# sebasv/lp

Measured on NVIDIA B200. Metric: ipm_iterations_per_s, higher is better.
Workload: dtype f64

## Files before the change

lp_b200/csrc/cholesky.cu:

```cuda
#include <nccl.h>

#include <algorithm>
#include <cstring>
#include <mutex>
#include <type_traits>

#include "dist_schedule.hpp"
#include "kernels.hpp"
#include "panel_factor.cuh"

namespace lpb {

namespace {

constexpr int NB = 128;
constexpr int LDS = NB + 1;
constexpr int TRSM_ROWS = 64;

__global__ void __launch_bounds__(512)
potf2_kernel(double* __restrict__ Mat, int64_t ldm, int k0, int nb, int* __restrict__ info) {
  extern __shared__ double S[];
  double* diag = S + NB * LDS;
  const int tx = threadIdx.x, ty = threadIdx.y, tid = ty * 32 + tx;
  double* blk = Mat + (int64_t)k0 * ldm + k0;
  for (int i = ty; i < nb; i += 16)
    for (int k = tx; k <= i; k += 32) S[i * LDS + k] = blk[(int64_t)i * ldm + k];
  __syncthreads();

  for (int j = 0; j < nb; ++j) {
    const double ajj = S[j * LDS + j];
    if (!(ajj > 0.0) || !isfinite(ajj)) {
      if (tid == 0 && *info == 0) *info = k0 + j + 1;
      for (int i = j + tid; i < nb; i += 512) diag[i] = __longlong_as_double(0x7ff8000000000000ll);
      break;
    }
    const double d = sqrt(ajj);
    if (tid == 0) diag[j] = d;
    if (tid < nb - j - 1) S[(j + 1 + tid) * LDS + j] /= d;
    __syncthreads();
    for (int i = j + 1 + ty; i < nb; i += 16) {
      const double lij = S[i * LDS + j];
      for (int k = j + 1 + tx; k <= i; k += 32) S[i * LDS + k] -= lij * S[k * LDS + j];
    }
    __syncthreads();
  }
  __syncthreads();
  for (int i = ty; i < nb; i += 16)
    for (int k = tx; k <= i; k += 32) blk[(int64_t)i * ldm + k] = (k == i) ? diag[i] : S[i * LDS + k];
}

constexpr int SB = 16;
constexpr int NSB = NB / SB;
constexpr int XDP = SB + 1;
constexpr int TWP = 9;

__device__ __forceinline__ void complete_block_inverse(double* S, const double* rdiag, double* Tw, int tid) {
  const int lane = tid & 31, warp = tid >> 5;
  const int b = warp >> 1, h = warp & 1;
  const int ii = lane & 15, cg = lane >> 4;
  double* tw = Tw + warp * SB * TWP;
  for (int d = 1; d < NSB; ++d) {
    if (b < NSB - d) {
      const int j = b, i = b + d;
      const int ccb = 8 * h + 4 * cg;
      double acc[4] = {0.0, 0.0, 0.0, 0.0};
      const double* lrow = S + (i * SB + ii) * LDS;
#pragma unroll
      for (int l = 0; l < SB; ++l) {
        const double lv = lrow[j * SB + l];
#pragma unroll
        for (int e = 0; e < 4; ++e) {
          const int cc = ccb + e;
          const double up = S[(j * SB + cc) * LDS + j * SB + l];
          const double xv = (l > cc) ? up : ((l == cc) ? rdiag[j * SB + cc] : 0.0);
          acc[e] += lv * xv;
        }
      }
      for (int k = j + 1; k < i; ++k) {
#pragma unroll
        for (int l = 0; l < SB; ++l) {
          const double lv = lrow[k * SB + l];
#pragma unroll
          for (int e = 0; e < 4; ++e) acc[e] += lv * S[(j * SB + ccb + e) * LDS + k * SB + l];
        }
      }
#pragma unroll
      for (int e = 0; e < 4; ++e) tw[ii * TWP + 4 * cg + e] = acc[e];
      __syncwarp();
      double o[4] = {0.0, 0.0, 0.0, 0.0};
#pragma unroll
// ... 1307 lines not shown
  return once.run([](int) -> int {
  LPB_TRY(set_smem(potf2_kernel, kPotf2Smem));
  LPB_TRY(set_smem(potf2_inv_kernel, kPotf2InvSmem));
  LPB_TRY(set_smem(trsm_kernel, kTrsmSmem));
  LPB_TRY(set_smem(trsm_blocked_kernel, kTrsmBlockedSmem));
  LPB_TRY(set_smem(trsm_dmma_blocked_kernel, kTrsmDmmaSmem));
  LPB_TRY(set_smem(trsv_diag_kernel<false, 1>, kTrsvSmem));
  LPB_TRY(set_smem(trsv_diag_kernel<false, 2>, kTrsvSmem));
  LPB_TRY(set_smem(trsv_diag_kernel<true, 1>, kTrsvSmem));
  LPB_TRY(set_smem(trsv_diag_kernel<true, 2>, kTrsvSmem));
  return LPB_OK;
  });
}

#define LPB_KCHECK(lc)             \
  do {                             \
    (lc).launches++;               \
    LPB_CUDA(cudaGetLastError());  \
  } while (0)

}

struct CholWs {
  int64_t nblk, ldy, off_y, off_flags, off_wt, off_xt, total;
  explicit CholWs(int64_t m) {
    nblk = ceil_div(m, NB);
    ldy = round_up(m, 2);
    off_y = nblk * NB * NB;
    off_flags = off_y + 2 * ldy;
    off_wt = off_flags + round_up(nblk, 2);
    off_xt = off_wt + nblk * 2 * NB * 2;
    total = off_xt + nblk * 2 * NB * 2;
  }
};

static int ensure_chol_ws(LaunchCtx& lc, int64_t m) {
  const int64_t need = CholWs(m).total;
  if (lc.chol_ws_cap >= need) return LPB_OK;
  if (lc.chol_ws) cudaFree(lc.chol_ws);
  lc.chol_ws = nullptr;
  lc.chol_ws_cap = 0;
  lc.linv_valid_m = -1;
  void* p = nullptr;
  LPB_CUDA(cudaMalloc(&p, sizeof(double) * (size_t)need));
  LPB_CUDA(cudaMemsetAsync(p, 0, sizeof(double) * (size_t)need, lc.stream));
  lc.chol_ws = static_cast<double*>(p);
  lc.chol_ws_cap = need;
  return LPB_OK;
}

static int finish_factor(LaunchCtx& lc, int64_t m, double* Mat, int64_t ldm) {
  if (lc.potf2_impl == 1) {
    lc.linv_valid_m = -1;
    lc.linv_mat = nullptr;
    return LPB_OK;
  }
  if (!lc.linv_full) {
    static PerDeviceOnce once;
    LPB_TRY(once.run([](int) -> int { return set_smem(linv_complete_kernel, kLinvCompleteSmem); }));
    linv_complete_kernel<<<(unsigned)ceil_div(m, NB), dim3(32, 16), kLinvCompleteSmem, lc.stream>>>(Mat, ldm, m, lc.chol_ws);
    LPB_KCHECK(lc);
    lc.linv_full = true;
  }
  lc.linv_valid_m = m;
  lc.linv_mat = Mat;
  return LPB_OK;
}

static int k_potrf_dist(LaunchCtx& lc, int64_t m, double* Mat, int64_t ldm);
static int k_potrf_dist2(LaunchCtx& lc, int64_t m, double* Mat, int64_t ldm);

static int k_potrf_lookahead(LaunchCtx& lc, int64_t m, double* Mat, int64_t ldm) {
  if (!lc.side_stream) {
    int lo = 0, hi = 0;
    LPB_CUDA(cudaDeviceGetStreamPriorityRange(&lo, &hi));
    LPB_CUDA(cudaStreamCreateWithPriority(&lc.side_stream, cudaStreamNonBlocking, hi));
    for (int e = 0; e < 2; ++e) {
      LPB_CUDA(cudaEventCreateWithFlags(&lc.ev_col[e], cudaEventDisableTiming));
      LPB_CUDA(cudaEventCreateWithFlags(&lc.ev_pan[e], cudaEventDisableTiming));
    }
  }
  const int T = (int)ceil_div(m, NB);
  lc.linv_full = false;
  auto nb_of = [&](int k) { return (int)((m - (int64_t)k * NB) < NB ? (m - (int64_t)k * NB) : NB); };
  auto potf2 = [&](int k, cudaStream_t st) -> int {
    potf2_inv_kernel<<<1, dim3(32, 16), kPotf2InvSmem, st>>>(Mat, ldm, k * NB, nb_of(k), lc.info_dev,
                                                             lc.chol_ws + (int64_t)k * NB * NB, 0);
    LPB_KCHECK(lc);
    return LPB_OK;
  };
  auto trsm = [&](int k) -> int {
    const int64_t rem = m - (int64_t)k * NB - nb_of(k);
    if (rem <= 0) return LPB_OK;
    trsm_dmma_blocked_kernel<<<(unsigned)ceil_div(rem, TBR), 256, kTrsmDmmaSmem, lc.stream>>>(
        Mat, ldm, k * NB, (int)m, lc.chol_ws + (int64_t)k * NB * NB);
    LPB_KCHECK(lc);
    return LPB_OK;
  };
  LPB_TRY(potf2(0, lc.stream));
  LPB_TRY(trsm(0));
  const int saved_cap = lc.update_grid_cap;
  int rc = LPB_OK;
  for (int k = 0; k + 1 < T && rc == LPB_OK; ++k) {
    const int64_t k0 = (int64_t)k * NB;
    cudaEvent_t ec = lc.ev_col[k & 1], ep = lc.ev_pan[k & 1];
    rc = k_trailing_update_part(lc, m, Mat, ldm, k0, NB, k + 1, 1, 1, 0);
    if (rc != LPB_OK) break;
    LPB_CUDA(cudaEventRecord(ec, lc.stream));
    LPB_CUDA(cudaStreamWaitEvent(lc.side_stream, ec, 0));
    rc = potf2(k + 1, lc.side_stream);
    if (rc != LPB_OK) break;
    LPB_CUDA(cudaEventRecord(ep, lc.side_stream));
    lc.update_grid_cap = kNumSMs - 1;
    rc = k_trailing_update_part(lc, m, Mat, ldm, k0, NB, k + 2, 0, 1, 0);
    lc.update_grid_cap = saved_cap;
    if (rc != LPB_OK) break;
    LPB_CUDA(cudaStreamWaitEvent(lc.stream, ep, 0));
    rc = trsm(k + 1);
  }
  lc.update_grid_cap = saved_cap;
  LPB_TRY(rc);
  return finish_factor(lc, m, Mat, ldm);
}

int k_potrf(LaunchCtx& lc, int64_t m, double* Mat, int64_t ldm, int syrk_impl) {
  LPB_TRY(configure_once());
  LPB_TRY(ensure_chol_ws(lc, m));
  if (lc.ws_m != m) {
    const CholWs ws(m);
    LPB_CUDA(cudaMemsetAsync(lc.chol_ws + ws.off_flags, 0, sizeof(double) * (size_t)(ws.total - ws.off_flags), lc.stream));
    lc.ws_m = m;
  }
  LPB_CUDA(cudaMemsetAsync(lc.info_dev, 0, sizeof(int), lc.stream));
  const bool dmma_update = lc.update_impl == 0 || lc.update_impl == 2 || lc.update_impl == 6;
  if (lc.world > 1 && lc.nccl_comm && lc.potrf_dist && syrk_impl == 0 && lc.trsm_impl == 0 && dmma_update &&
      lc.potf2_impl == 0 && m > NB && !(ldm & 1) && !(reinterpret_cast<uintptr_t>(Mat) & 15))
    return lc.potrf_dist == 2 ? k_potrf_dist2(lc, m, Mat, ldm) : k_potrf_dist(lc, m, Mat, ldm);
  if (lc.potrf_lookahead && syrk_impl == 0 && lc.trsm_impl == 0 && dmma_update && lc.potf2_impl == 0 &&
      !lc.sync_each_launch && m > 2 * NB && !(ldm & 1) && !(reinterpret_cast<uintptr_t>(Mat) & 15))
    return k_potrf_lookahead(lc, m, Mat, ldm);
  const int full_inverse = lc.trsm_impl == 2 ? 1 : 0;
  lc.linv_full = full_inverse != 0;
  for (int64_t k0 = 0; k0 < m; k0 += NB) {
    const int nb = (int)((m - k0) < NB ? (m - k0) : NB);
    const int64_t rem = m - k0 - nb;
    double* linv = lc.chol_ws + (k0 / NB) * NB * NB;
    if (lc.potf2_impl == 1)
      potf2_kernel<<<1, dim3(32, 16), kPotf2Smem, lc.stream>>>(Mat, ldm, (int)k0, nb, lc.info_dev);
    else
      potf2_inv_kernel<<<1, dim3(32, 16), kPotf2InvSmem, lc.stream>>>(Mat, ldm, (int)k0, nb, lc.info_dev, linv,
                                                                      full_inverse);
    LPB_KCHECK(lc);
    if (lc.sync_each_launch) LPB_CUDA(cudaStreamSynchronize(lc.stream));
    if (rem > 0) {
      if (syrk_impl == 1 || lc.trsm_impl == 1) {
        trsm_kernel<<<(unsigned)ceil_div(rem, TRSM_ROWS), dim3(32, 8), kTrsmSmem, lc.stream>>>(Mat, ldm, (int)k0, nb,
                                                                                               (int)m);
        LPB_KCHECK(lc);
      } else if (lc.trsm_impl == 2) {
        LPB_TRY(k_trsm_dmma(lc, m, Mat, ldm, k0, linv));
      } else if (lc.trsm_impl == 3 || (ldm & 1) || (reinterpret_cast<uintptr_t>(Mat) & 15)) {
        trsm_blocked_kernel<<<(unsigned)ceil_div(rem, TBR), 256, kTrsmBlockedSmem, lc.stream>>>(Mat, ldm, (int)k0,
                                                                                               (int)m, linv);
        LPB_KCHECK(lc);
      } else {
        trsm_dmma_blocked_kernel<<<(unsigned)ceil_div(rem, TBR), 256, kTrsmDmmaSmem, lc.stream>>>(Mat, ldm, (int)k0,
                                                                                                 (int)m, linv);
        LPB_KCHECK(lc);
      }
      if (lc.sync_each_launch) LPB_CUDA(cudaStreamSynchronize(lc.stream));
      if (syrk_impl == 1 || lc.update_impl == 1)
        LPB_TRY(k_trailing_update_simple(lc, m, Mat, ldm, k0, nb));
      else
        LPB_TRY(k_trailing_update_dmma(lc, m, Mat, ldm, k0, nb));
      if (lc.sync_each_launch) LPB_CUDA(cudaStreamSynchronize(lc.stream));
    }
  }
  return finish_factor(lc, m, Mat, ldm);
}

static int ensure_dist_streams(LaunchCtx& lc) {
  if (!lc.side_stream) {
    int lo = 0, hi = 0;
    LPB_CUDA(cudaDeviceGetStreamPriorityRange(&lo, &hi));
    LPB_CUDA(cudaStreamCreateWithPriority(&lc.side_stream, cudaStreamNonBlocking, hi));
    for (int e = 0; e < 2; ++e) {
      LPB_CUDA(cudaEventCreateWithFlags(&lc.ev_col[e], cudaEventDisableTiming));
      LPB_CUDA(cudaEventCreateWithFlags(&lc.ev_pan[e], cudaEventDisableTiming));
    }
  }
  for (int e = 0; e < 4; ++e)
    if (!lc.ev_dist[e]) LPB_CUDA(cudaEventCreateWithFlags(&lc.ev_dist[e], cudaEventDisableTiming));
  return LPB_OK;
}

constexpr int kPushCtasPerPeer = 4;
constexpr int kRingHeaderDoubles = 128;
struct PeerPush {
  double* dst[LaunchCtx::kMaxPeers - 1];
  unsigned long long* flag[LaunchCtx::kMaxPeers - 1];
  int n;
};
__global__ void __launch_bounds__(256)
peer_push_kernel(const double* __restrict__ src, int64_t count2, PeerPush pp, unsigned long long value,
// ... 507 lines not shown
```

lp_b200/csrc/common.cuh:

```cuda
#pragma once
#include <cuda_runtime.h>
#include <cstdint>
#include <cstdio>
#include <cstring>
#include <mutex>

#include "../../include/lpb200.h"

namespace lpb {

void set_last_error(const char* fmt, ...);
const char* get_last_error();

#define LPB_CUDA(call)                                                                         \
  do {                                                                                         \
    cudaError_t e__ = (call);                                                                  \
    if (e__ != cudaSuccess) {                                                                  \
      ::lpb::set_last_error("%s:%d %s -> %s", __FILE__, __LINE__, #call, cudaGetErrorString(e__)); \
      return LPB_ERR_CUDA;                                                                     \
    }                                                                                          \
  } while (0)

#define LPB_TRY(call)              \
  do {                             \
    int rc__ = (call);             \
    if (rc__ != LPB_OK) return rc__; \
  } while (0)

constexpr int kNumSMs = 148;

constexpr int kMaxDevices = 64;
struct PerDeviceOnce {
  std::mutex mu;
  bool done[kMaxDevices] = {};
  template <class F>
  int run(F&& f) {
    int dev = 0;
    LPB_CUDA(cudaGetDevice(&dev));
    if (dev < 0 || dev >= kMaxDevices) return f(dev);
    std::lock_guard<std::mutex> g(mu);
    if (done[dev]) return LPB_OK;
    const int rc = f(dev);
    if (rc == LPB_OK) done[dev] = true;
    return rc;
  }
};

inline int64_t round_up(int64_t v, int64_t a) { return (v + a - 1) / a * a; }
inline int64_t ceil_div(int64_t a, int64_t b) { return (a + b - 1) / b; }

constexpr int kMaxRedVals = 8;
constexpr int kMaxRedBlocks = 1024;
enum RedOp : int { kRedSum = 0, kRedMin = 1 };

struct LaunchCtx {
  cudaStream_t stream = nullptr;
  int64_t launches = 0;
  double* red_partials = nullptr;
  double* red_out = nullptr;
  double* red_host = nullptr;
  unsigned long long* fault_dev = nullptr;
  double* gemv_partials = nullptr;
  int64_t gemv_partials_cap = 0;
  double* chol_ws = nullptr;
  int64_t chol_ws_cap = 0;
  int64_t ws_m = -1;
  int64_t linv_valid_m = -1;
  const double* linv_mat = nullptr;
  bool linv_full = false;
  int solve_epoch = 0;
  int solve_impl = 0;
  int sync_each_launch = 0;
  int syrk_flush_blocks = 32;
  int syrk_tail_split = 1;
  double* syrk_ws = nullptr;
  int64_t syrk_ws_cap = 0;
  int syrk_chain = 0;
  int potf2_impl = 0;
  int trsm_impl = 0, update_impl = 0;
  int solve_grid_cap = 0;
  void* nccl_comm = nullptr;
  int rank = 0, world = 1;
  int potrf_dist = 2;
  double* panel_buf = nullptr;
  int64_t panel_buf_cap = 0;
  int potrf_lookahead = 1;
  cudaStream_t side_stream = nullptr;
  cudaEvent_t ev_col[2] = {nullptr, nullptr}, ev_pan[2] = {nullptr, nullptr};
  bool launch_on_side = false;
  cudaEvent_t ev_dist[4] = {nullptr, nullptr, nullptr, nullptr};
  double* panel_slot[2] = {nullptr, nullptr};
  int64_t panel_slot_cap = 0;
  static constexpr int kMaxPeers = 8;
  double* ring_base = nullptr;
  int64_t ring_slot_doubles = 0;
  int ring_slots = 0;
  double* peer_base[kMaxPeers] = {};
  bool peer_mapped = false;
  bool peer_ready = false;
  uint32_t dist_epoch = 0;
  int update_grid_cap = 0;
  int* info_dev = nullptr;
  int* info_host = nullptr;
};

}
```

lp_b200/csrc/dist_schedule.hpp:

```cpp
#pragma once
#include <cmath>

#if defined(__CUDACC__)
#define LPB_SCHED_HD __host__ __device__
#else
#define LPB_SCHED_HD
#endif

namespace lpb {

struct OwnedCols {
  int G, f, n;
  LPB_SCHED_HD int before(int l) const { return l * (n - f) - G * (l * (l - 1) / 2); }
  LPB_SCHED_HD int count() const {
    if (f >= n) return 0;
    const int nown = (n - f + G - 1) / G;
    return before(nown);
  }
  LPB_SCHED_HD void decode(int t, int* ti, int* tj) const {
    const double a = 0.5 * G, b = (n - f) + 0.5 * G;
    const double disc = b * b - 4.0 * a * t;
    int l = static_cast<int>((b - sqrt(disc > 0.0 ? disc : 0.0)) / (2.0 * a));
    if (l < 0) l = 0;
    while (l > 0 && before(l) > t) --l;
    while (before(l + 1) <= t) ++l;
    *tj = f + l * G;
    *ti = *tj + (t - before(l));
  }
  static LPB_SCHED_HD OwnedCols make(int G, int rank, int tile0, int ntr) {
    OwnedCols o;
    o.G = G;
    o.f = ((rank - tile0) % G + G) % G;
    o.n = ntr;
    return o;
  }
};

template <class Ops>
int potrf_dist_schedule(int T, int G, int me, Ops& ops) {
  int pending = -1;
  for (int k = 0; k < T; ++k) {
    const int owner = k % G;
    int rc;
    if (owner == me && (rc = ops.factor_panel(k)) != 0) return rc;
    if ((rc = ops.broadcast(k, owner)) != 0) return rc;
    if (owner != me && (rc = ops.store_panel(k)) != 0) return rc;
    if (pending >= 0) {
      if ((rc = ops.update_owned(pending, pending + 2)) != 0) return rc;
      pending = -1;
    }
    if (k + 1 < T) {
      if ((k + 1) % G == me) {
        if ((rc = ops.update_column(k, k + 1)) != 0) return rc;
        pending = k;
      } else if ((rc = ops.update_owned(k, k + 1)) != 0) {
        return rc;
      }
    }
  }
  return 0;
}

enum { kEvSmall = 0, kEvPotf2 = 2, kNumDistEvents = 4 };

template <class Ops>
int potrf_dist_schedule2(int T, int G, int me, Ops& ops) {
#define LPB_S2(call)            \
  do {                          \
    const int rc__ = (call);    \
    if (rc__ != 0) return rc__; \
  } while (0)
  int pending = -1;
  for (int k = 0; k < T; ++k) {
    const int owner = k % G;
    if (owner == me) {
      if (k == 0)
        LPB_S2(ops.potf2(0, 0));
      else
        LPB_S2(ops.wait(kEvPotf2 + (k & 1), 0));
      LPB_S2(ops.trsm(k));
    }
    if (k + 1 < T) {
      LPB_S2(ops.bcast_small(k, owner));
      LPB_S2(ops.record(kEvSmall + (k & 1), 0));
    }
    LPB_S2(ops.bcast_large(k, owner));
    if (pending >= 0) {
      LPB_S2(ops.update_owned(pending, pending + 2));
      if (pending % G != me) LPB_S2(ops.unpack(pending));
      pending = -1;
    }
    if (k + 1 < T && (k + 1) % G == me) {
      LPB_S2(ops.wait(kEvSmall + (k & 1), 1));
      LPB_S2(ops.update_diag(k, k + 1, 1));
      LPB_S2(ops.potf2(k + 1, 1));
      LPB_S2(ops.record(kEvPotf2 + ((k + 1) & 1), 1));
      LPB_S2(ops.update_col_below(k, k + 1));
      pending = k;
    } else {
      if (k + 1 < T) LPB_S2(ops.update_owned(k, k + 1));
// ... 10 lines not shown
```

lp_b200/csrc/dmma_gemm.cu:

```cuda
#include <cuda.h>

#include "dist_schedule.hpp"
#include "kernels.hpp"

namespace lpb {

namespace {

constexpr int BM = 128, BN = 128, BK = 16;
constexpr int kStages = 5;
constexpr int kLead = 3;
constexpr int kFlushBlocks = 128;
constexpr int kConsumerWarps = 8;
constexpr int kThreads = kConsumerWarps * 32;
constexpr uint32_t kTileBytes = BM * BK * 8;
constexpr uint32_t kDBytes = BK * 8;
constexpr uint32_t kSmemA = 0;
constexpr uint32_t kSmemB = kSmemA + kStages * kTileBytes;
constexpr uint32_t kSmemD = kSmemB + kStages * kTileBytes;
constexpr uint32_t kSmemBar = kSmemD + kStages * kDBytes;
constexpr uint32_t kSmemTotal = kSmemBar + 2 * kStages * 8;
constexpr uint32_t kSmemAlloc = kSmemTotal + 1024;

template <int MODE, int VAR>
// ... 37 lines not shown
      "{\n\t.reg .pred p;\n\t"
      "mbarrier.try_wait.parity.shared::cta.b64 p, [%1], %2;\n\t"
      "selp.u32 %0, 1, 0, p;\n\t}"
      : "=r"(ok)
      : "r"(bar), "r"(parity)
      : "memory");
  return ok;
}
__device__ __forceinline__ void mbar_wait(uint32_t bar, uint32_t parity) {
  if (mbar_try_wait(bar, parity)) return;
  const long long t0 = clock64();
  while (!mbar_try_wait(bar, parity)) {
    if (clock64() - t0 > 8000000000ll) __trap();
  }
}
__device__ __forceinline__ void tma_load_2d(uint32_t dst, const CUtensorMap* tm, int c0, int c1, uint32_t bar) {
  asm volatile(
      "cp.async.bulk.tensor.2d.shared::cluster.global.mbarrier::complete_tx::bytes [%0], [%1, {%2, %3}], [%4];" ::"r"(
          dst),
      "l"(reinterpret_cast<uint64_t>(tm)), "r"(c0), "r"(c1), "r"(bar)
      : "memory");
}
__device__ __forceinline__ double2 lds_v2(uint32_t addr) {
  double2 v;
  asm volatile("ld.volatile.shared.v2.f64 {%0, %1}, [%2];" : "=d"(v.x), "=d"(v.y) : "r"(addr));
  return v;
}
__device__ __forceinline__ void cp_async_16(uint32_t dst, const void* src) {
  asm volatile("cp.async.cg.shared.global [%0], [%1], 16;" ::"r"(dst), "l"(src) : "memory");
}
__device__ __forceinline__ void cp_async_commit() { asm volatile("cp.async.commit_group;" ::: "memory"); }
__device__ __forceinline__ void cp_async_wait_all() { asm volatile("cp.async.wait_group 0;" ::: "memory"); }
__device__ __forceinline__ void dmma884(double& c0, double& c1, double a, double b) {
  asm("mma.sync.aligned.m8n8k4.row.col.f64.f64.f64.f64 {%0, %1}, {%2}, {%3}, {%0, %1};"
      : "+d"(c0), "+d"(c1)
      : "d"(a), "d"(b));
}

__device__ __forceinline__ void tri_decode(int L, int* ti, int* tj) {
  int i = static_cast<int>((sqrt(8.0 * static_cast<double>(L) + 1.0) - 1.0) * 0.5);
  while (i * (i + 1) / 2 > L) --i;
  while ((i + 1) * (i + 2) / 2 <= L) ++i;
  *ti = i;
  *tj = L - i * (i + 1) / 2;
}

constexpr int kBand = 12;
__device__ __forceinline__ void band_decode(int L, int ntr, int* ti, int* tj) {
  int row, col;
  tri_decode(L, &row, &col);
  const int r0 = (row / kBand) * kBand;
  const int r1 = r0 + kBand < ntr ? r0 + kBand : ntr;
  const int h = r1 - r0;
  int off = L - r0 * (r0 + 1) / 2;
  const int rect = (r0 + 1) * h;
  if (off < rect) {
    *tj = off / h;
    *ti = r0 + off % h;
    return;
  }
  off -= rect;
  int c = r0 + 1, hh = h - 1;
  while (off >= hh) {
    off -= hh;
    ++c;
    --hh;
  }
  *tj = c;
  *ti = c + off;
}

struct LoadCursor {
  int L, kb, row_i, row_j, stage;
  int kb_lo, kb_n;
  uint32_t phase;
};

struct TailSplit {
  int n_full, nsplit;
  double* ws;
};

enum { MODE_SYRK = 0, MODE_UPDATE = 1, MODE_TRSM = 2 };
enum { SHAPE_TRI = 0, SHAPE_COL = 1, SHAPE_OWNED = 2, SHAPE_COLB = 3 };

template <int MODE, bool SCALE, int VAR = 0>
__global__ void __maxnreg__(255)
syrk_dmma_kernel(const __grid_constant__ CUtensorMap tmA, const __grid_constant__ CUtensorMap tmB,
                 double* __restrict__ C, int64_t ldc, int m_total, int tile0, int ntr, int k_begin, int nkb,
                 int col_origin, int shape, OwnedCols own, int p_row0, TailSplit ts) {
  using P = Plan<MODE, VAR>;
  constexpr bool FLUSH = (VAR & 16) == 0;
  constexpr int NS = P::kNS, LEAD = P::kLd;
  constexpr bool CPF = P::kCpf;
  extern __shared__ uint8_t smem_raw[];
  const uint32_t smem_base = (smem_u32(smem_raw) + 1023u) & ~1023u;
  const uint32_t sA = smem_base + P::kA, sB = smem_base + P::kB, sD = smem_base + P::kD, sC = smem_base + P::kC;
  const uint32_t bar_full = smem_base + P::kBar, bar_empty = bar_full + NS * 8;
  const uint32_t bar_cfull = bar_empty + NS * 8, bar_cempty = bar_cfull + 8;
  const uint32_t sF = smem_base + P::kF + threadIdx.x * 16u;

  const int warp = threadIdx.x >> 5, lane = threadIdx.x & 31;
  if (threadIdx.x == 0) {
    for (int s = 0; s < NS; ++s) {
      mbar_init(bar_full + s * 8, 1);
      mbar_init(bar_empty + s * 8, kConsumerWarps);
    }
    mbar_init(bar_cfull, 1);
    mbar_init(bar_cempty, kConsumerWarps);
    asm volatile("fence.mbarrier_init.release.cluster;" ::: "memory");
  }
  __syncthreads();

  constexpr bool SPLIT = MODE == MODE_SYRK && FLUSH && (VAR & 32) != 0;
  const int ntiles_whole = (MODE == MODE_TRSM || shape == SHAPE_COL) ? ntr
                     : (shape == SHAPE_COLB ? ntr - 1 : (shape == SHAPE_OWNED ? own.count() : ntr * (ntr + 1) / 2));
  const int ntiles = SPLIT ? ts.n_full + (ntiles_whole - ts.n_full) * ts.nsplit : ntiles_whole;
  auto item = [&](int I, int* L, int* part, int* kb_lo, int* kb_n) {
    if (!SPLIT || I < ts.n_full) {
      *L = I;
      *part = -1;
      *kb_lo = 0;
      *kb_n = nkb;
    } else {
      const int q = I - ts.n_full;
      *L = ts.n_full + q / ts.nsplit;
      *part = q % ts.nsplit;
      *kb_lo = (int)((int64_t)nkb * *part / ts.nsplit);
      *kb_n = (int)((int64_t)nkb * (*part + 1) / ts.nsplit) - *kb_lo;
    }
  };
  const bool is_producer = threadIdx.x == 0;
  constexpr uint32_t kBytes = 2 * kTileBytes + (SCALE ? kDBytes : 0);

  auto decode = [&](int L, int* ti, int* tj) {
    if (MODE == MODE_TRSM || shape == SHAPE_COL) {
      *ti = L;
      *tj = 0;
    } else if (shape == SHAPE_COLB) {
      *ti = L + 1;
      *tj = 0;
    } else if (shape == SHAPE_OWNED) {
      own.decode(L, ti, tj);
    } else if (MODE == MODE_SYRK) {
      band_decode(L, ntr, ti, tj);
    } else {
      tri_decode(L, ti, tj);
    }
  };

  LoadCursor pc;
  pc.L = blockIdx.x;
  pc.kb = 0;
  pc.stage = 0;
  pc.phase = 0;
  pc.row_i = pc.row_j = 0;
  pc.kb_lo = 0;
  pc.kb_n = nkb;
  auto cursor_tile = [&]() {
    if (pc.L < ntiles) {
      int ti, tj, Lt, part;
      item(pc.L, &Lt, &part, &pc.kb_lo, &pc.kb_n);
      decode(Lt, &ti, &tj);
      pc.row_i = (tile0 + ti) * BM;
      pc.row_j = MODE == MODE_TRSM ? 0 : (tile0 + tj) * BN;
    }
  };
  auto produce_one = [&]() {
    if (pc.L >= ntiles) return;
    mbar_wait(bar_empty + pc.stage * 8, pc.phase ^ 1u);
    const uint32_t full = bar_full + pc.stage * 8;
    mbar_expect_tx(full, kBytes);
    const int k = k_begin + (pc.kb_lo + pc.kb) * BK;
    int ra = pc.row_i, rb = pc.row_j;
    if (MODE == MODE_UPDATE && p_row0 >= 0) {
      ra -= p_row0;
      rb -= p_row0;
      if (ra == BM) ra = 0;
      if (rb == BN) rb = 0;
    }
    tma_load_2d(sA + pc.stage * kTileBytes, &tmA, k, ra, full);
    if (MODE == MODE_TRSM)
      tma_load_2d(sB + pc.stage * kTileBytes, &tmB, (pc.kb_lo + pc.kb) * BK, 0, full);
    else
      tma_load_2d(sB + pc.stage * kTileBytes, &tmA, k, rb, full);
    if (SCALE) tma_load_2d(sD + pc.stage * kDBytes, &tmB, k, 0, full);
    if (++pc.stage == NS) {
      pc.stage = 0;
      pc.phase ^= 1u;
    }
    if (++pc.kb == pc.kb_n) {
      pc.kb = 0;
      pc.L += gridDim.x;
      cursor_tile();
    }
  };
  int c_next = blockIdx.x;
  int c_issued = 0;
  auto produce_c = [&]() {
    if (!CPF || c_next >= ntiles) return;
    if (c_issued > 0) mbar_wait(bar_cempty, static_cast<uint32_t>((c_issued - 1) & 1));
    int ti, tj;
    decode(c_next, &ti, &tj);
    const int r0 = (tile0 + ti) * BM, c0 = (tile0 + tj) * BN;
    mbar_expect_tx(bar_cfull, 8 * kTileBytes);
#pragma unroll
    for (int b = 0; b < 8; ++b) tma_load_2d(sC + b * kTileBytes, &tmB, c0 + b * BK, r0, bar_cfull);
    c_next += gridDim.x;
    ++c_issued;
  };
  if (is_producer) {
    cursor_tile();
    produce_c();
    for (int i = 0; i < LEAD; ++i) produce_one();
  }

  int stage = 0;
  uint32_t phase = 0;
  const int wm = warp >> 2, wn = warp & 3;
  const int g = lane >> 2, t = lane & 3;
  const uint32_t offA = static_cast<uint32_t>(wm * 64 + g) * 128u;
  const uint32_t offB = static_cast<uint32_t>(wn * 32 + g) * 128u;
  const uint32_t sw[2] = {static_cast<uint32_t>(((2 * t + 0) ^ g) << 4), static_cast<uint32_t>(((2 * t + 1) ^ g) << 4)};
  const uint32_t dof[2] = {static_cast<uint32_t>((2 * t + 0) << 4), static_cast<uint32_t>((2 * t + 1) << 4)};

  const int fblocks = MODE == MODE_SYRK && col_origin >= 32 ? col_origin : kFlushBlocks;
  const int fstride = fblocks >> 3;
// ... 279 lines not shown
  if (d)
    LPB_TRY(make_tmap(&tmD, d, 1, (uint64_t)n, (uint64_t)round_up(n, 2), 1, BK, false));
  else
    tmD = tmA;
  const int ntr = (int)ceil_div(m, BM);
  const int nkb = (int)ceil_div(n, BK);
  if (lc.syrk_chain) {
    if (d) return launch_dmma<MODE_SYRK, true, 16>(lc, tmA, tmD, Cmat, ldc, (int)m, 0, ntr, 0, nkb, 0);
    return launch_dmma<MODE_SYRK, false, 16>(lc, tmA, tmD, Cmat, ldc, (int)m, 0, ntr, 0, nkb, 0);
  }
  const int fb = lc.syrk_flush_blocks;
  TailSplit ts{0, 1, nullptr};
  const int ntiles = ntr * (ntr + 1) / 2;
  const int rem = ntiles % kNumSMs;
  if (lc.syrk_tail_split && ntiles > kNumSMs && rem > 0 && 4 * rem <= 3 * kNumSMs && nkb >= 64 && !(m & 1)) {
    int best_s = 1;
    double best = 1.0;
    for (int sp = 2; sp <= 8; ++sp) {
      const double len = (double)ceil_div((int64_t)rem * sp, (int64_t)kNumSMs) / sp + 0.01 * sp;
      if (len < best - 1e-9) {
        best = len;
        best_s = sp;
      }
    }
    if (best_s > 1) {
      const int64_t need = (int64_t)rem * best_s * BM * BN;
      if (lc.syrk_ws_cap < need) {
        if (lc.syrk_ws) LPB_CUDA(cudaFree(lc.syrk_ws));
        lc.syrk_ws = nullptr;
        lc.syrk_ws_cap = 0;
        void* p = nullptr;
        LPB_CUDA(cudaMalloc(&p, sizeof(double) * (size_t)need));
        lc.syrk_ws = static_cast<double*>(p);
        lc.syrk_ws_cap = need;
      }
      ts = TailSplit{ntiles - rem, best_s, lc.syrk_ws};
    }
  }
  if (ts.nsplit > 1) {
    if (d)
      LPB_TRY((launch_dmma<MODE_SYRK, true, 32>(lc, tmA, tmD, Cmat, ldc, (int)m, 0, ntr, 0, nkb, fb, SHAPE_TRI, OwnedCols{1, 0, 0}, -1, ts)));
    else
      LPB_TRY((launch_dmma<MODE_SYRK, false, 32>(lc, tmA, tmD, Cmat, ldc, (int)m, 0, ntr, 0, nkb, fb, SHAPE_TRI, OwnedCols{1, 0, 0}, -1, ts)));
  } else if (d) {
    LPB_TRY((launch_dmma<MODE_SYRK, true>(lc, tmA, tmD, Cmat, ldc, (int)m, 0, ntr, 0, nkb, fb)));
  } else {
    LPB_TRY((launch_dmma<MODE_SYRK, false>(lc, tmA, tmD, Cmat, ldc, (int)m, 0, ntr, 0, nkb, fb)));
  }
  if (ts.nsplit > 1) {
    syrk_tail_fixup_kernel<<<rem, 256, 0, lc.stream>>>(Cmat, ldc, (int)m, ntr, ts);
    lc.launches++;
    LPB_CUDA(cudaGetLastError());
  }
  return LPB_OK;
}

int k_trailing_update_dmma(LaunchCtx& lc, int64_t m, double* Mat, int64_t ldm, int64_t k0, int64_t kb) {
  const int64_t row0 = k0 + kb;
  if (row0 >= m) return LPB_OK;
  if ((row0 % BM) || (kb % BK) || (ldm & 1) || (reinterpret_cast<uintptr_t>(Mat) & 15)) {
    set_last_error("trailing_update_dmma: panel origin must be a multiple of %d, width a multiple of %d", BM, BK);
    return LPB_ERR_BAD_ARGUMENT;
  }
  CUtensorMap tm;
  LPB_TRY(make_tmap(&tm, Mat, (uint64_t)m, (uint64_t)m, (uint64_t)ldm, BM, BK, true));
  const int ntr = (int)ceil_div(m - row0, BM);
  if (lc.update_impl == 2)
    return launch_dmma<MODE_UPDATE, false, 1>(lc, tm, tm, Mat, ldm, (int)m, (int)(row0 / BM), ntr, (int)k0,
                                              (int)(kb / BK), 0);
  if (lc.update_impl == 3)
    return launch_dmma<MODE_UPDATE, false, 2>(lc, tm, tm, Mat, ldm, (int)m, (int)(row0 / BM), ntr, (int)k0,
                                              (int)(kb / BK), 0);
  if (lc.update_impl == 4)
    return launch_dmma<MODE_UPDATE, false, 4>(lc, tm, tm, Mat, ldm, (int)m, (int)(row0 / BM), ntr, (int)k0,
                                              (int)(kb / BK), 0);
  if (lc.update_impl == 5)
    return launch_dmma<MODE_UPDATE, false, 6>(lc, tm, tm, Mat, ldm, (int)m, (int)(row0 / BM), ntr, (int)k0,
                                              (int)(kb / BK), 0);
  return launch_dmma<MODE_UPDATE, false>(lc, tm, tm, Mat, ldm, (int)m, (int)(row0 / BM), ntr, (int)k0, (int)(kb / BK),
                                         0);
}

int k_trailing_update_part(LaunchCtx& lc, int64_t m, double* Mat, int64_t ldm, int64_t k0, int64_t kb, int tile0,
                           int single_col, int own_mod, int own_rem, const double* packed, int64_t packed_rows) {
  int ntr = (int)ceil_div(m, BM) - tile0;
  if (ntr <= 0) return LPB_OK;
  if ((kb % BK) || (ldm & 1) || (reinterpret_cast<uintptr_t>(Mat) & 15) || (int64_t)tile0 * BM < k0 + kb) {
    set_last_error("trailing_update_part: bad panel / tile origin");
    return LPB_ERR_BAD_ARGUMENT;
  }
  CUtensorMap tm, tmc;
  int k_begin = (int)k0, p_row0 = -1;
  LPB_TRY(make_tmap(&tmc, Mat, (uint64_t)m, (uint64_t)m, (uint64_t)ldm, BM, BK, true));
  if (packed) {
    LPB_TRY(make_tmap(&tm, packed, (uint64_t)packed_rows, (uint64_t)BN, (uint64_t)BN, BM, BK, true));
    k_begin = 0;
    p_row0 = (int)k0;
  } else {
    tm = tmc;
  }
  int shape = SHAPE_TRI;
  if (single_col == 1) shape = SHAPE_COL;
  if (single_col == 2) {
    shape = SHAPE_COL;
    ntr = 1;
  }
  if (single_col == 3) shape = SHAPE_COLB;
  if (!single_col && own_mod > 1) shape = SHAPE_OWNED;
  const OwnedCols own = shape == SHAPE_OWNED ? OwnedCols::make(own_mod, own_rem, tile0, ntr) : OwnedCols{1, 0, 0};
  if (lc.update_impl == 2)
    return launch_dmma<MODE_UPDATE, false, 1>(lc, tm, tm, Mat, ldm, (int)m, tile0, ntr, k_begin, (int)(kb / BK), 0, shape,
                                              own, p_row0);
  if (lc.update_impl == 6)
    return launch_dmma<MODE_UPDATE, false, 8>(lc, tm, tmc, Mat, ldm, (int)m, tile0, ntr, k_begin, (int)(kb / BK), 0,
                                              shape, own, p_row0);
  return launch_dmma<MODE_UPDATE, false>(lc, tm, tm, Mat, ldm, (int)m, tile0, ntr, k_begin, (int)(kb / BK), 0, shape, own,
                                         p_row0);
}

int k_trsm_dmma(LaunchCtx& lc, int64_t m, double* Mat, int64_t ldm, int64_t k0, const double* Linv) {
  const int64_t row0 = k0 + BN;
  if (row0 >= m) return LPB_OK;
  if ((row0 % BM) || (ldm & 1) || (reinterpret_cast<uintptr_t>(Mat) & 15) || (reinterpret_cast<uintptr_t>(Linv) & 15)) {
    set_last_error("trsm_dmma: panel origin must be a multiple of %d", BM);
    return LPB_ERR_BAD_ARGUMENT;
  }
  CUtensorMap tm, tl;
  LPB_TRY(make_tmap(&tm, Mat, (uint64_t)m, (uint64_t)m, (uint64_t)ldm, BM, BK, true));
  LPB_TRY(make_tmap(&tl, Linv, (uint64_t)BN, (uint64_t)BN, (uint64_t)BN, BN, BK, true));
  const int ntr = (int)ceil_div(m - row0, BM);
  return launch_dmma<MODE_TRSM, false>(lc, tm, tl, Mat, ldm, (int)m, (int)(row0 / BM), ntr, (int)k0, BN / BK, (int)k0);
}

__global__ void __launch_bounds__(256)
dmma_peak_kernel(double* out, int iters, double a0, double b0) {
  double c[32][2];
#pragma unroll
  for (int i = 0; i < 32; ++i) c[i][0] = c[i][1] = threadIdx.x * 1e-3 + i;
  const double a = a0 + threadIdx.x * 1e-9, b = b0;
  for (int it = 0; it < iters; ++it) {
#pragma unroll
    for (int i = 0; i < 32; ++i) dmma884(c[i][0], c[i][1], a, b);
  }
  double s = 0.0;
#pragma unroll
  for (int i = 0; i < 32; ++i) s += c[i][0] + c[i][1];
  if (s == 12345.678) out[0] = s;
}

int k_dmma_peak(LaunchCtx& lc, double seconds, double* tflops) {
  if (seconds < 0.05) seconds = 0.05;
  if (seconds > 2.0) seconds = 2.0;
  const int iters = 4000;
  const double flop_per_launch = 2.0 * 256 * 32 * iters * 8.0 * kNumSMs;
  cudaEvent_t e0, e1;
  LPB_CUDA(cudaEventCreate(&e0));
  LPB_CUDA(cudaEventCreate(&e1));
  auto run = [&](int launches, float* ms) -> int {
    LPB_CUDA(cudaEventRecord(e0, lc.stream));
    for (int i = 0; i < launches; ++i) dmma_peak_kernel<<<kNumSMs, 256, 0, lc.stream>>>(lc.red_partials, iters, 1.0000001, 1e-9);
    LPB_CUDA(cudaEventRecord(e1, lc.stream));
    LPB_CUDA(cudaEventSynchronize(e1));
    LPB_CUDA(cudaEventElapsedTime(ms, e0, e1));
    lc.launches += launches;
    return LPB_OK;
  };
  float ms = 0.f;
  int rc = run(4, &ms);
  if (rc == LPB_OK) {
    int launches = (int)(seconds * 1e3 / (ms / 4.0 > 1e-3 ? ms / 4.0 : 1e-3));
    if (launches < 8) launches = 8;
    if (launches > 4000) launches = 4000;
    rc = run(launches, &ms);
    if (rc == LPB_OK && tflops) *tflops = flop_per_launch * launches / (ms * 1e-3) * 1e-12;
  }
  cudaEventDestroy(e0);
  cudaEventDestroy(e1);
  return rc;
}

template <bool ACCUM>
__global__ void __launch_bounds__(256)
syrk_simple_kernel(int m_total, int row_origin, int k_begin, int k_end, const double* __restrict__ A, int64_t lda,
                   const double* __restrict__ d, double* __restrict__ C, int64_t ldc) {
  __shared__ double sa[16][65], sb[16][65];
  const int bi = blockIdx.y, bj = blockIdx.x;
  if (bj > bi) return;
  const int tx = threadIdx.x & 15, ty = threadIdx.x >> 4, tid = threadIdx.x;
  double acc[4][4];
#pragma unroll
  for (int i = 0; i < 4; ++i)
#pragma unroll
// ... 62 lines not shown
```

lp_b200/csrc/kernels.hpp:

```cpp
#pragma once
#include "common.cuh"

namespace lpb {

struct RedSpec {
  int nvals = 0;
  int nblocks[kMaxRedVals] = {0};
  int op[kMaxRedVals] = {0};
};
int reduce_finalize(LaunchCtx& lc, const RedSpec& spec);
int fetch_scalars(LaunchCtx& lc, int nvals);

int k_fill(LaunchCtx& lc, double* p, int64_t n, double v);
int k_copy(LaunchCtx& lc, double* dst, const double* src, int64_t n);
int k_dinv(LaunchCtx& lc, int64_t n, const double* x, const double* z, double* dinv);

int k_rhat(LaunchCtx& lc, int64_t n, int mode, double eta, double gm, double a2, double s, const double* x,
           const double* z, const double* rD, const double* dx, const double* dz, double* xs, double* r1);

int k_assemble_delta_n(LaunchCtx& lc, int64_t n, double d_tau, const double* u, const double* p, const double* xs,
                       const double* x, const double* z, double* dx, double* dz, int val_base, int* nblocks);
int k_assemble_delta_m(LaunchCtx& lc, int64_t m, double d_tau, const double* v, const double* q, double* dy);
int k_step(LaunchCtx& lc, int64_t n, double alpha, int clamp, double* x, const double* dx);
int k_extract_x(LaunchCtx& lc, int64_t n, double tau, const double* x, const double* c, double* xo, int val,
                int* nblocks);

int k_resid_p(LaunchCtx& lc, int64_t m, double tau, const double* b, const double* t, const double* y, double* rP,
              int val_base, int* nblocks);
int k_sym_fwd_rhs(LaunchCtx& lc, int64_t m, double eta, const double* rP, const double* b, const double* t0,
                  const double* t1, double* rhs0, double* rhs1, int with_pq);
int k_refine_rhs(LaunchCtx& lc, int64_t m, double eta, const double* rP, const double* b, const double* au,
                 const double* ap, double* rho0, double* rho1, int with_pq);
int k_add_inplace(LaunchCtx& lc, int64_t count, const double* x, double* y);
int k_dots_m(LaunchCtx& lc, int64_t m, const double* b, const double* v, const double* q, int with_pq, int val_base,
             int* nblocks);

int k_gemv_n(LaunchCtx& lc, int64_t m, int64_t n, const double* A, int64_t lda, const double* dinv, const double* w0,
             const double* w1, double* t0, double* t1, int nrhs);
int k_gemv_t_partials(LaunchCtx& lc, int64_t m, int64_t n, const double* A, int64_t lda, const double* v0,
                      const double* v1, int nrhs, int* nchunks);
struct TailCols {
  int64_t nd;
  const int* col_row;
  const double* col_val;
  const double* v0;
  const double* v1;
};
int k_gemv_t_raw(LaunchCtx& lc, int64_t n, int nchunks, int nrhs, double* out0, double* out1);
int k_resid_d(LaunchCtx& lc, int64_t n, int nchunks, double tau, const double* c, const double* z, const double* x,
              double* rD, int val_base, int* nblocks, const TailCols* tail = nullptr);
int k_sym_back(LaunchCtx& lc, int64_t n, int nchunks, int with_pq, const double* dinv, const double* r1,
               const double* c, double* u, double* p, int val_base, int* nblocks, const TailCols* tail = nullptr);

int k_syrk_dmma(LaunchCtx& lc, int64_t m, int64_t n, const double* A, int64_t lda, const double* d, double* Cmat,
                int64_t ldc);
int k_trailing_update_dmma(LaunchCtx& lc, int64_t m, double* Mat, int64_t ldm, int64_t k0, int64_t kb);
int k_trailing_update_part(LaunchCtx& lc, int64_t m, double* Mat, int64_t ldm, int64_t k0, int64_t kb, int tile0,
                           int single_col, int own_mod, int own_rem, const double* packed = nullptr,
                           int64_t packed_rows = 0);
int k_trsm_dmma(LaunchCtx& lc, int64_t m, double* Mat, int64_t ldm, int64_t k0, const double* Linv);
int k_dmma_peak(LaunchCtx& lc, double seconds, double* tflops);
int k_syrk_simple(LaunchCtx& lc, int64_t m, int64_t n, const double* A, int64_t lda, const double* d, double* Cmat,
                  int64_t ldc);
int k_trailing_update_simple(LaunchCtx& lc, int64_t m, double* Mat, int64_t ldm, int64_t k0, int64_t kb);

int k_potrf(LaunchCtx& lc, int64_t m, double* Mat, int64_t ldm, int syrk_impl);
int k_potrf_dist_reserve(LaunchCtx& lc, int64_t m);
int k_peer_export(LaunchCtx& lc, int64_t m, unsigned char* handle_out, int* state_out);
int k_peer_import(LaunchCtx& lc, const unsigned char* handles, int world);
void k_peer_release(LaunchCtx& lc);
void k_peer_abandon(LaunchCtx& lc);
void k_peer_free_process();
int k_potrs(LaunchCtx& lc, int64_t m, const double* L, int64_t ldm, double* B, int nrhs, bool use_linv);

int k_fill_normal(LaunchCtx& lc, double* A, int64_t rows, int64_t cols, int64_t lda, int64_t row0, int64_t col0,
                  uint64_t seed);
int k_fill_vec(LaunchCtx& lc, double* v, int64_t count, int64_t idx0, uint64_t seed, int kind, double lo, double hi,
               int64_t neg_below);
int k_slack_identity(LaunchCtx& lc, double* A, int64_t rows, int64_t cols, int64_t lda, int64_t col0, int64_t n0);
int k_add_vec(LaunchCtx& lc, double* out, const double* a, const double* b, int64_t count, int64_t count_b);
int k_col_structure(LaunchCtx& lc, const double* A, int64_t m, int64_t n, int64_t lda, int* nnz, int* row, double* val);
int k_diag_add(LaunchCtx& lc, int64_t m, double* M, int64_t ldm, const int* col, const double* val, const double* dinv);
int k_diag_shift(LaunchCtx& lc, int64_t m, double* M, int64_t ldm, double delta);
int k_slack_add(LaunchCtx& lc, int64_t m, const int* col, const double* val, const double* dinv, const double* w0,
                const double* w1, double* t0, double* t1, int nrhs);
int64_t tri_packed_doubles(int64_t m);
int k_tri_pack(LaunchCtx& lc, double* M, int64_t ldm, int64_t m, double* buf, bool pack);
int k_diff(LaunchCtx& lc, const double* a, const double* b, int64_t rows, int64_t cols, int64_t ld, int lower_only,
           unsigned long long* out_dev3);
int k_checksum(LaunchCtx& lc, const double* v, int64_t rows, int64_t cols, int64_t ld, int lower_only,
               unsigned long long* out_dev);

}
```

lp_b200/csrc/lpb_api.cu:

```cuda
#include <nccl.h>

#include <algorithm>
#include <chrono>
#include <cmath>
#include <cstdlib>
#include <mutex>
#include <new>
#include <string>
#include <vector>

#include "ipm_driver.hpp"
#include "kernels.hpp"

namespace lpb {
int64_t gemv_t_partials_doubles(int64_t m, int64_t n);
int batched_launch(int64_t batch, int m, int n, const double* dA, const double* db, const double* dc,
                   const lpb_options& o, double* dx, double* dfun, int64_t* dit, int32_t* dst, cudaStream_t stream);
}

using namespace lpb;

enum Phase { PH_SYRK = 0, PH_POTRF, PH_SOLVE, PH_SWEEP, PH_VEC, PH_COMM, PH_COUNT };

struct PhaseRec {
// ... 1286 lines not shown
  *out = c->prof;
  return LPB_OK;
}

int64_t lpb_launch_count(lpb_ctx* c) { return c ? c->lc.launches : 0; }

int lpb_measure_dmma_peak(lpb_ctx* c, double seconds, double* tflops_out) {
  if (!c || !tflops_out) return LPB_ERR_BAD_ARGUMENT;
  return k_dmma_peak(c->lc, seconds, tflops_out);
}

int lpb_set_option(lpb_ctx* c, const char* key, int64_t value) {
  if (!c || !key) return LPB_ERR_BAD_ARGUMENT;
  const std::string k(key);
  if (k == "syrk_impl") {
    if (value != 0 && value != 1) return LPB_ERR_BAD_ARGUMENT;
    c->syrk_impl = (int)value;
    return LPB_OK;
  }
  if (k == "solve_impl") {
    if (value < 0 || value > 3) return LPB_ERR_BAD_ARGUMENT;
    c->lc.solve_impl = (int)value;
    return LPB_OK;
  }
  if (k == "trsm_impl" || k == "update_impl") {
    if (value < 0 || value > 6) return LPB_ERR_BAD_ARGUMENT;
    (k == "trsm_impl" ? c->lc.trsm_impl : c->lc.update_impl) = (int)value;
    return LPB_OK;
  }
  if (k == "syrk_tail_split") {
    c->lc.syrk_tail_split = value != 0;
    return LPB_OK;
  }
  if (k == "syrk_chain") {
    c->lc.syrk_chain = value != 0;
    return LPB_OK;
  }
  if (k == "peer_panels") {
    if (value > 0 && !c->lc.peer_mapped) return LPB_ERR_BAD_ARGUMENT;
    if (value < 0)
      k_peer_abandon(c->lc);
    else
      c->lc.peer_ready = value != 0;
    return LPB_OK;
  }
  if (k == "syrk_flush_blocks") {
    if (value < 32 || value > (1 << 20) || (value & (value - 1))) return LPB_ERR_BAD_ARGUMENT;
    c->lc.syrk_flush_blocks = (int)value;
    return LPB_OK;
  }
  if (k == "potf2_impl") {
    if (value < 0 || value > 1) return LPB_ERR_BAD_ARGUMENT;
    c->lc.potf2_impl = (int)value;
    if (value == 1) c->lc.trsm_impl = 1;
    return LPB_OK;
  }
  if (k == "solve_grid_cap") {
    if (value < 0) return LPB_ERR_BAD_ARGUMENT;
    c->lc.solve_grid_cap = (int)value;
    return LPB_OK;
  }
  if (k == "refine") {
    if (value < 0 || value > 4) return LPB_ERR_BAD_ARGUMENT;
    c->refine = (int)value;
    return LPB_OK;
  }
  if (k == "refine_max") {
    if (value < 0 || value > 8) return LPB_ERR_BAD_ARGUMENT;
    c->refine_max = (int)value;
    return LPB_OK;
  }
  if (k == "regularize") {
    c->regularize = value != 0;
    return LPB_OK;
  }
  if (k == "structure") {
    c->use_structure = value != 0;
    return c->has_problem ? analyze_structure(c) : LPB_OK;
  }
  if (k == "potrf_lookahead") {
    c->lc.potrf_lookahead = value != 0;
    return LPB_OK;
  }
  if (k == "packed_allreduce") {
    c->packed_allreduce = value != 0;
    return LPB_OK;
  }
  if (k == "potrf_dist") {
    if (value < 0 || value > 2) return LPB_ERR_BAD_ARGUMENT;
    c->lc.potrf_dist = (int)value;
    return LPB_OK;
  }
  if (k == "potrf_verify") {
    c->potrf_verify = (int)value;
    return LPB_OK;
  }
  if (k == "sync_each_launch") {
    c->lc.sync_each_launch = (int)value;
    return LPB_OK;
  }
  if (k == "check_replicas") {
    c->check_replicas = value != 0;
    return LPB_OK;
  }
  if (k == "profile") {
    c->profile = value != 0;
    return LPB_OK;
  }
  set_last_error("unknown option '%s'", key);
  return LPB_ERR_BAD_ARGUMENT;
}

}
```

Baseline: 4.003.

## Group Cholesky panels into strips factored on a side stream alongside bulk updates

Replaces the one-panel lookahead in the blocked Cholesky with a grouped schedule. Each group of G panels is factored as a strip on a side stream with R SMs, while the main stream runs the trailing update of the previous group with the remaining SMs. A simple cost model picks R, and the update kernel gains band and column-limited owned shapes to support this. This is meant to hide the serial panel factor/TRSM latency for large matrices (T>=64). In exchange it adds extra launches, ordering dependencies and the risk of a poor SM split.

```diff
diff --git a/lp_b200/csrc/cholesky.cu b/lp_b200/csrc/cholesky.cu
--- a/lp_b200/csrc/cholesky.cu
+++ b/lp_b200/csrc/cholesky.cu
@@ -6,6 +6,7 @@
 #include <type_traits>
 
 #include "dist_schedule.hpp"
+#include "potrf_group.hpp"
 #include "kernels.hpp"
 #include "panel_factor.cuh"
 
@@ -1479,44 +1480,53 @@
   }
   const int T = (int)ceil_div(m, NB);
   lc.linv_full = false;
-  auto nb_of = [&](int k) { return (int)((m - (int64_t)k * NB) < NB ? (m - (int64_t)k * NB) : NB); };
-  auto potf2 = [&](int k, cudaStream_t st) -> int {
-    potf2_inv_kernel<<<1, dim3(32, 16), kPotf2InvSmem, st>>>(Mat, ldm, k * NB, nb_of(k), lc.info_dev,
-                                                             lc.chol_ws + (int64_t)k * NB * NB, 0);
-    LPB_KCHECK(lc);
-    return LPB_OK;
-  };
-  auto trsm = [&](int k) -> int {
-    const int64_t rem = m - (int64_t)k * NB - nb_of(k);
-    if (rem <= 0) return LPB_OK;
-    trsm_dmma_blocked_kernel<<<(unsigned)ceil_div(rem, TBR), 256, kTrsmDmmaSmem, lc.stream>>>(
-        Mat, ldm, k * NB, (int)m, lc.chol_ws + (int64_t)k * NB * NB);
-    LPB_KCHECK(lc);
-    return LPB_OK;
-  };
-  LPB_TRY(potf2(0, lc.stream));
-  LPB_TRY(trsm(0));
-  const int saved_cap = lc.update_grid_cap;
-  int rc = LPB_OK;
-  for (int k = 0; k + 1 < T && rc == LPB_OK; ++k) {
-    const int64_t k0 = (int64_t)k * NB;
-    cudaEvent_t ec = lc.ev_col[k & 1], ep = lc.ev_pan[k & 1];
-    rc = k_trailing_update_part(lc, m, Mat, ldm, k0, NB, k + 1, 1, 1, 0);
-    if (rc != LPB_OK) break;
-    LPB_CUDA(cudaEventRecord(ec, lc.stream));
-    LPB_CUDA(cudaStreamWaitEvent(lc.side_stream, ec, 0));
-    rc = potf2(k + 1, lc.side_stream);
-    if (rc != LPB_OK) break;
-    LPB_CUDA(cudaEventRecord(ep, lc.side_stream));
-    lc.update_grid_cap = kNumSMs - 1;
-    rc = k_trailing_update_part(lc, m, Mat, ldm, k0, NB, k + 2, 0, 1, 0);
-    lc.update_grid_cap = saved_cap;
-    if (rc != LPB_OK) break;
-    LPB_CUDA(cudaStreamWaitEvent(lc.stream, ep, 0));
-    rc = trsm(k + 1);
-  }
-  lc.update_grid_cap = saved_cap;
-  LPB_TRY(rc);
+  struct Ops {
+    LaunchCtx& lc;
+    int64_t m;
+    double* Mat;
+    int64_t ldm;
+    int T;
+    int nb_of(int k) const { return (int)((m - (int64_t)k * NB) < NB ? (m - (int64_t)k * NB) : NB); }
+    cudaStream_t st(int side) const { return side ? lc.side_stream : lc.stream; }
+    cudaEvent_t ev(int e) const { return e >= kEvGroupPan ? lc.ev_pan[e - kEvGroupPan] : lc.ev_col[e - kEvGroupCol]; }
+    int potf2(int k, int side) {
+      potf2_inv_kernel<<<1, dim3(32, 16), kPotf2InvSmem, st(side)>>>(Mat, ldm, k * NB, nb_of(k), lc.info_dev,
+                                                                     lc.chol_ws + (int64_t)k * NB * NB, 0);
+      LPB_KCHECK(lc);
+      return LPB_OK;
+    }
+    int trsm(int k, int side) {
+      const int64_t rem = m - (int64_t)k * NB - nb_of(k);
+      if (rem <= 0) return LPB_OK;
+      trsm_dmma_blocked_kernel<<<(unsigned)ceil_div(rem, TBR), 256, kTrsmDmmaSmem, st(side)>>>(
+          Mat, ldm, k * NB, (int)m, lc.chol_ws + (int64_t)k * NB * NB);
+      LPB_KCHECK(lc);
+      return LPB_OK;
+    }
+    int update(int p, int np, int tile0, int ncols, int side, int cap) {
+      const bool tri = tile0 + ncols >= T;
+      const int shape = ncols == 1 ? 1 : (tri ? (np > 1 ? 4 : 0) : 0);
+      const int saved_cap = lc.update_grid_cap;
+      lc.update_grid_cap = cap;
+      lc.launch_on_side = side != 0;
+      const int rc = k_trailing_update_part(lc, m, Mat, ldm, (int64_t)p * NB, (int64_t)np * NB, tile0, shape, 1, 0,
+                                            nullptr, 0, tri || ncols == 1 ? 0 : ncols);
+      lc.update_grid_cap = saved_cap;
+      lc.launch_on_side = false;
+      return rc;
+    }
+    int record(int e, int side) {
+      LPB_CUDA(cudaEventRecord(ev(e), st(side)));
+      return LPB_OK;
+    }
+    int wait(int e, int side) {
+      LPB_CUDA(cudaStreamWaitEvent(st(side), ev(e), 0));
+      return LPB_OK;
+    }
+  } ops{lc, m, Mat, ldm, T};
+  const int G = lc.update_impl != 0 ? 1 : (lc.potrf_group > 0 ? lc.potrf_group : (T >= 64 ? 8 : 1));
+  PotrfGroupSchedule<Ops> sched{T, G, lc.potrf_side_sms, ops};
+  LPB_TRY(sched.run());
   return finish_factor(lc, m, Mat, ldm);
 }
 
diff --git a/lp_b200/csrc/common.cuh b/lp_b200/csrc/common.cuh
--- a/lp_b200/csrc/common.cuh
+++ b/lp_b200/csrc/common.cuh
@@ -85,6 +85,8 @@
   double* panel_buf = nullptr;
   int64_t panel_buf_cap = 0;
   int potrf_lookahead = 1;
+  int potrf_group = 0;
+  int potrf_side_sms = 0;
   cudaStream_t side_stream = nullptr;
   cudaEvent_t ev_col[2] = {nullptr, nullptr}, ev_pan[2] = {nullptr, nullptr};
   bool launch_on_side = false;
diff --git a/lp_b200/csrc/dist_schedule.hpp b/lp_b200/csrc/dist_schedule.hpp
--- a/lp_b200/csrc/dist_schedule.hpp
+++ b/lp_b200/csrc/dist_schedule.hpp
@@ -11,11 +11,12 @@
 
 struct OwnedCols {
   int G, f, n;
+  int ncols = 1 << 30;
   LPB_SCHED_HD int before(int l) const { return l * (n - f) - G * (l * (l - 1) / 2); }
   LPB_SCHED_HD int count() const {
     if (f >= n) return 0;
     const int nown = (n - f + G - 1) / G;
-    return before(nown);
+    return before(nown < ncols ? nown : ncols);
   }
   LPB_SCHED_HD void decode(int t, int* ti, int* tj) const {
     const double a = 0.5 * G, b = (n - f) + 0.5 * G;
diff --git a/lp_b200/csrc/dmma_gemm.cu b/lp_b200/csrc/dmma_gemm.cu
--- a/lp_b200/csrc/dmma_gemm.cu
+++ b/lp_b200/csrc/dmma_gemm.cu
@@ -143,7 +143,7 @@
 };
 
 enum { MODE_SYRK = 0, MODE_UPDATE = 1, MODE_TRSM = 2 };
-enum { SHAPE_TRI = 0, SHAPE_COL = 1, SHAPE_OWNED = 2, SHAPE_COLB = 3 };
+enum { SHAPE_TRI = 0, SHAPE_COL = 1, SHAPE_OWNED = 2, SHAPE_COLB = 3, SHAPE_BAND = 4 };
 
 template <int MODE, bool SCALE, int VAR = 0>
 __global__ void __maxnreg__(255)
@@ -203,7 +203,7 @@
       *tj = 0;
     } else if (shape == SHAPE_OWNED) {
       own.decode(L, ti, tj);
-    } else if (MODE == MODE_SYRK) {
+    } else if (MODE == MODE_SYRK || shape == SHAPE_BAND) {
       band_decode(L, ntr, ti, tj);
     } else {
       tri_decode(L, ti, tj);
@@ -649,7 +649,8 @@
 }
 
 int k_trailing_update_part(LaunchCtx& lc, int64_t m, double* Mat, int64_t ldm, int64_t k0, int64_t kb, int tile0,
-                           int single_col, int own_mod, int own_rem, const double* packed, int64_t packed_rows) {
+                           int single_col, int own_mod, int own_rem, const double* packed, int64_t packed_rows,
+                           int ncols) {
   int ntr = (int)ceil_div(m, BM) - tile0;
   if (ntr <= 0) return LPB_OK;
   if ((kb % BK) || (ldm & 1) || (reinterpret_cast<uintptr_t>(Mat) & 15) || (int64_t)tile0 * BM < k0 + kb) {
@@ -673,8 +674,10 @@
     ntr = 1;
   }
   if (single_col == 3) shape = SHAPE_COLB;
-  if (!single_col && own_mod > 1) shape = SHAPE_OWNED;
-  const OwnedCols own = shape == SHAPE_OWNED ? OwnedCols::make(own_mod, own_rem, tile0, ntr) : OwnedCols{1, 0, 0};
+  if (single_col == 4) shape = SHAPE_BAND;
+  if (!single_col && (own_mod > 1 || ncols > 0)) shape = SHAPE_OWNED;
+  OwnedCols own = shape == SHAPE_OWNED ? OwnedCols::make(own_mod, own_rem, tile0, ntr) : OwnedCols{1, 0, 0};
+  if (ncols > 0) own.ncols = ncols;
   if (lc.update_impl == 2)
     return launch_dmma<MODE_UPDATE, false, 1>(lc, tm, tm, Mat, ldm, (int)m, tile0, ntr, k_begin, (int)(kb / BK), 0, shape,
                                               own, p_row0);
diff --git a/lp_b200/csrc/kernels.hpp b/lp_b200/csrc/kernels.hpp
--- a/lp_b200/csrc/kernels.hpp
+++ b/lp_b200/csrc/kernels.hpp
@@ -57,7 +57,7 @@
 int k_trailing_update_dmma(LaunchCtx& lc, int64_t m, double* Mat, int64_t ldm, int64_t k0, int64_t kb);
 int k_trailing_update_part(LaunchCtx& lc, int64_t m, double* Mat, int64_t ldm, int64_t k0, int64_t kb, int tile0,
                            int single_col, int own_mod, int own_rem, const double* packed = nullptr,
-                           int64_t packed_rows = 0);
+                           int64_t packed_rows = 0, int ncols = 0);
 int k_trsm_dmma(LaunchCtx& lc, int64_t m, double* Mat, int64_t ldm, int64_t k0, const double* Linv);
 int k_dmma_peak(LaunchCtx& lc, double seconds, double* tflops);
 int k_syrk_simple(LaunchCtx& lc, int64_t m, int64_t n, const double* A, int64_t lda, const double* d, double* Cmat,
diff --git a/lp_b200/csrc/lpb_api.cu b/lp_b200/csrc/lpb_api.cu
--- a/lp_b200/csrc/lpb_api.cu
+++ b/lp_b200/csrc/lpb_api.cu
@@ -1392,6 +1392,16 @@
     c->lc.potrf_lookahead = value != 0;
     return LPB_OK;
   }
+  if (k == "potrf_group") {
+    if (value < 0 || value > 64) return LPB_ERR_BAD_ARGUMENT;
+    c->lc.potrf_group = (int)value;
+    return LPB_OK;
+  }
+  if (k == "potrf_side_sms") {
+    if (value < 0 || value > 147) return LPB_ERR_BAD_ARGUMENT;
+    c->lc.potrf_side_sms = (int)value;
+    return LPB_OK;
+  }
   if (k == "packed_allreduce") {
     c->packed_allreduce = value != 0;
     return LPB_OK;
diff --git a/lp_b200/csrc/potrf_group.hpp b/lp_b200/csrc/potrf_group.hpp
--- /dev/null
+++ b/lp_b200/csrc/potrf_group.hpp
@@ -0,0 +1,97 @@
+#pragma once
+
+namespace lpb {
+
+constexpr int kGroupSMs = 148;
+enum { kEvGroupCol = 0, kEvGroupPan = 2, kNumGroupEvents = 4 };
+
+struct GroupCost {
+  static int waves(long long n, int sms) { return (int)((n + sms - 1) / sms); }
+  static long long strip_tiles(int T, int c0, int c1) {
+    long long n = 0;
+    for (int j = c0; j < c1; ++j) n += T - j;
+    return n;
+  }
+  static double strip(int T, int p1, int p2, int R) {
+    double t = 0.0;
+    for (int k = p1; k < p2; ++k) t += 1.8 + 0.5 * waves(2LL * (T - k - 1), R) + waves(strip_tiles(T, k + 1, p2), R);
+    return t;
+  }
+  static double bulk(int T, int np, int p2, int S) {
+    const long long n = (long long)(T - p2) * (T - p2 + 1) / 2;
+    return waves(n, S) * (0.2 + 0.8 * np);
+  }
+  static int side_sms(int T, int np, int p1, int p2) {
+    if (p2 >= T) return 0;
+    int best = 0;
+    double best_t = 0.0;
+    for (int R = 1; R < kGroupSMs; ++R) {
+      const double s = strip(T, p1, p2, R), b = bulk(T, np, p2, kGroupSMs - R);
+      const double t = s > b ? s : b;
+      if (s <= b && (best == 0 || t < best_t)) {
+        best = R;
+        best_t = t;
+      }
+    }
+    return best;
+  }
+};
+
+template <class Ops, class Cost = GroupCost>
+struct PotrfGroupSchedule {
+  int T, G, side_sms_opt;
+  Ops& ops;
+
+  int panels(int kb, int ke, int ce) {
+    int rc;
+    if ((rc = ops.potf2(kb, 0)) || (rc = ops.trsm(kb, 0))) return rc;
+    for (int k = kb; k + 1 < ke; ++k) {
+      const int e = k & 1;
+      if ((rc = ops.update(k, 1, k + 1, 1, 0, 0)) || (rc = ops.record(kEvGroupCol + e, 0)) ||
+          (rc = ops.wait(kEvGroupCol + e, 1)) || (rc = ops.potf2(k + 1, 1)) || (rc = ops.record(kEvGroupPan + e, 1)))
+        return rc;
+      if (k + 2 < ce && (rc = ops.update(k, 1, k + 2, ce - (k + 2), 0, kGroupSMs - 1))) return rc;
+      if ((rc = ops.wait(kEvGroupPan + e, 0)) || (rc = ops.trsm(k + 1, 0))) return rc;
+    }
+    return 0;
+  }
+
+  int strip_side(int p1, int p2, int R) {
+    int rc;
+    for (int k = p1; k < p2; ++k) {
+      if ((rc = ops.potf2(k, 1)) || (rc = ops.trsm(k, 1))) return rc;
+      if (k + 1 < p2 && (rc = ops.update(k, 1, k + 1, p2 - (k + 1), 1, R))) return rc;
+    }
+    return 0;
+  }
+
+  int side_sms(int np, int p1, int p2) const {
+    if (side_sms_opt > 0) return p2 < T ? (side_sms_opt < kGroupSMs ? side_sms_opt : kGroupSMs - 1) : 0;
+    return Cost::side_sms(T, np, p1, p2);
+  }
+
+  int run() {
+    if (G <= 1 || side_sms(G, G, 2 * G) == 0) return panels(0, T, T);
+    int rc, p0 = 0, p1 = G;
+    if ((rc = panels(0, p1, p1))) return rc;
+    for (int g = 0;; ++g) {
+      const int p2 = p1 + G < T ? p1 + G : T;
+      const int R = side_sms(p1 - p0, p1, p2);
+      if (R == 0) {
+        if ((rc = ops.update(p0, p1 - p0, p1, T - p1, 0, 0))) return rc;
+        return panels(p1, T, T);
+      }
+      const int e = g & 1;
+      if ((rc = ops.update(p0, p1 - p0, p1, p2 - p1, 0, 0)) ||
+          (rc = ops.record(kEvGroupCol + e, 0)) || (rc = ops.wait(kEvGroupCol + e, 1)) ||
+          (rc = strip_side(p1, p2, R)) || (rc = ops.record(kEvGroupPan + e, 1)) ||
+          (rc = ops.update(p0, p1 - p0, p2, T - p2, 0, kGroupSMs - R)) ||
+          (rc = ops.wait(kEvGroupPan + e, 0)))
+        return rc;
+      p0 = p1;
+      p1 = p2;
+    }
+  }
+};
+
+}
```

Result: faster. 4.053, median of 6 (+1.2%).
